# MarioniLab/sarlacc

Hardware: AMD Instinct MI355X
Metric: GCUPS (quality-aware pairwise DP cell updates/s), adaptor_align .Call level (higher is better)
Workload: dtype f64; 1 GPU; adaptorAlign: 1000000 x 2000 bp mockReads-like reads per GPU vs 30 bp adaptor, local quality DP + traceback + 1 section, go=5 ge=1; reads_per_gpu=1000000, read_len=2000, adaptor_len=30, resident_format=2-bit packed bases + 1-bit non-ACGT mask + 1 B quality per base

## Files before the change

### sarlacc_amd/csrc/align.hip

```cpp
#include "align_host.hpp"

#include "../../include/sarlacc_amd.h"

#include <algorithm>
#include <cmath>
#include <cstdlib>
#include <cstring>
#include <limits>

namespace sarlacc {

constexpr int NGMAX = 4;
constexpr int NGMAX2 = 8;
constexpr int NWAVES = 4;
constexpr int RING = 128;
constexpr int RING_MIRROR = 8;
constexpr int RING_SLOT = 256;
constexpr int MAX_REF = 1024;

struct AlignArgs {
    const uint8_t* seq;
    const uint8_t* nmask;
    const uint8_t* qual;
    const int64_t* off;
// ... 14 lines not shown
    const int32_t* sec_e;
    int nsec;
    int32_t* sec_so;
    int32_t* sec_wo;
    void* dirs;
    unsigned long long dirs_per_wave;
    int snap_head, snap_win;
    int* badqual;
    int read_base;
    long long sec_stride;
    uint8_t* aln_ref;
    uint8_t* aln_qry;
    int32_t* aln_len;
    int32_t* edits;
    int wide_maxlen;
    double* wide_bnd;
    int wide_band;
    int* wide_redo;
    const int* wide_list;
    const int* loc_tab;
    const int* loc_rz;
    int loc_GO, loc_GE, loc_D;
    int loc_framed;
    int loc_force;
    double loc_unit, loc_slack, loc_top;
    int* loc_redo;
    int* loc_stats;
    int* loc_out;
    uint8_t* loc_cls;
    int* loc_ccount;
    int* loc_over;
    const int* read_list;
    int bad_done;
};

using mask_t = unsigned long long;
typedef const double __attribute__((address_space(3))) lds_cdouble;
typedef const uint16_t __attribute__((address_space(3))) lds_cu16;
typedef const int __attribute__((address_space(3))) lds_cint;

__device__ __forceinline__ int sel32(int if0, int if1, mask_t m) {
    int r;
    asm("v_cndmask_b32 %0, %1, %2, %3" : "=v"(r) : "v"(if0), "v"(if1), "s"(m));
    return r;
}
__device__ __forceinline__ uint32_t push_bit(uint32_t pk, mask_t m) {
    uint32_t r;
    mask_t carry_out;
    asm("v_addc_co_u32 %0, %1, %2, %2, %3" : "=v"(r), "=s"(carry_out) : "v"(pk), "s"(m));
    return r;
}
__device__ __forceinline__ int hi32(double v) { return static_cast<int>(__double_as_longlong(v) >> 32); }
__device__ __forceinline__ int lo32(double v) { return static_cast<int>(__double_as_longlong(v)); }
__device__ __forceinline__ double mk64(int hi, int lo) {
    return __longlong_as_double((static_cast<long long>(hi) << 32) | static_cast<unsigned int>(lo));
}

template <int ROWF>
__device__ __forceinline__ int lane_shr1(int v, int keep) {
    if (ROWF == 1) return __builtin_amdgcn_update_dpp(keep, v, 0x111 , 0xf, 0xf, false);
    if (ROWF == 2) return __builtin_amdgcn_update_dpp(keep, v, 0x112 , 0xf, 0xf, false);
    return __builtin_amdgcn_update_dpp(v, v, 0x138 , 0xf, 0xf, false);
}
template <int ROWF>
__device__ __forceinline__ double lane_shr1(double v, double keep) {
    return mk64(lane_shr1<ROWF>(hi32(v), hi32(keep)), lane_shr1<ROWF>(lo32(v), lo32(keep)));
}

template <int K>
struct TbSteps { static constexpr int value = (8 / K) > 0 ? 8 / K : 1; };
template <int K>
struct TbStore { using type = uint32_t; };
template <>
struct TbStore<16> { using type = unsigned long long; };

template <bool B>
struct Flag { static constexpr bool value = B; };
template <int V>
struct Int { static constexpr int value = V; };

constexpr int SNAP_P = 64;
static inline int snap_head(int R) { return R + R / 4 + 4; }
static inline int snap_win(int R, int W) { return (SNAP_P + snap_head(R) + W + 7) / 8 * 8; }

constexpr int LOC_NEG = -(1 << 29);
constexpr int LOC_NEG_FRAMED = -(1 << 30);
constexpr int LOC_FRAME_KMIN = 8;
constexpr int LOC_WAVES = 4;
constexpr int LOC_STATS = 6;
constexpr int LOC_NCLS = 32;

struct WinPlan { int ts, want, need; };
__device__ __forceinline__ WinPlan window_plan(const AlignArgs& A, int imax, int lo_x2, int hi_x2) {
    const int lo = (lo_x2 >> 1) + 1, hi = (hi_x2 >> 1) + 1;
    const double f_low = static_cast<double>(imax) * A.loc_unit - A.loc_slack;
    const double over = floor((A.loc_top - f_low) / A.GE) + 1.0;
    const int wc = A.R + (over > 0.0 ? static_cast<int>(fmin(over, 1.0e6)) : 0);
    const int r0 = lo - wc;
    const int ts = r0 < 8 ? 0 : (r0 & ~7);
    return {ts, hi, hi + A.W + 1 - ts};
}

__global__ void __launch_bounds__(256) k_loc_order(const uint8_t* cls, long long n, int* ctl, int* perm) {
    __shared__ int s_cnt[LOC_NCLS], s_base[LOC_NCLS];
    const int t = threadIdx.x;
    if (t < LOC_NCLS) s_cnt[t] = 0;
    __syncthreads();
    const long long read = static_cast<long long>(blockIdx.x) * 256 + t;
    const int c = read < n ? min(static_cast<int>(cls[read]), LOC_NCLS - 1) : 0;
    int rank = 0;
    if (c) rank = atomicAdd(&s_cnt[c], 1);
    __syncthreads();
    if (t < LOC_NCLS) {
        int taller = 0;
        for (int x = t + 1; x < LOC_NCLS; ++x) taller += ctl[x];
        const int mine = t ? s_cnt[t] : 0;
        s_base[t] = taller + (mine ? atomicAdd(&ctl[LOC_NCLS + t], mine) : 0);
        if (blockIdx.x == 0 && t == 0) perm[0] = taller;
    }
    __syncthreads();
    if (c) perm[2 + s_base[c] + rank] = static_cast<int>(read);
}

template <int K, int MODE, bool LOCAL, int ROWF, int KLAST, bool PENSEL>
__global__ void __launch_bounds__(64 * NWAVES, MODE >= 5 ? LOC_WAVES : (MODE == 3 && ROWF != 2) ? 6 : 5) k_align(const AlignArgs A) {
    constexpr bool ROW16 = ROWF != 0;
    constexpr int NG = ROWF == 2 ? NGMAX2 : NGMAX;
    constexpr int SLOT = ROWF == 2 ? RING + RING_MIRROR : RING_SLOT;
    constexpr int UNR = TbSteps<K>::value;
    constexpr int CELLS = UNR * K;
    using Word = typename TbStore<K>::type;
    constexpr bool ADDC = sizeof(Word) == 4;
    extern __shared__ __align__(256) unsigned char smem[];
    static_assert(RING * sizeof(uint16_t) == 256 && RING + RING_MIRROR <= RING_SLOT, "ring addressing assumes 256 B of ring inside a 512 B slot");
    constexpr int RING_BYTES = NWAVES * NG * SLOT * static_cast<int>(sizeof(uint16_t));
    static_assert(RING_BYTES % 8 == 0 && (SLOT * sizeof(uint16_t)) % 8 == 0, "table and 8-byte ring stores stay aligned");
    double* const s_tab = reinterpret_cast<double*>(smem + RING_BYTES);
    const int lds0 = static_cast<int>(reinterpret_cast<size_t>((__attribute__((address_space(3))) unsigned char*)smem));

    const int lane = threadIdx.x & 63;
    const int wave = __builtin_amdgcn_readfirstlane(threadIdx.x >> 6);
    const int W = A.W, R = A.R;
    auto lane_of = [&](int gg, int jj) -> int { return ROWF == 2 ? ((gg >> 1) << 4) + (jj << 1) + (gg & 1) : gg * W + jj; };
    const int g = ROWF == 2 ? (((lane >> 4) << 1) | (lane & 1)) : lane / W;
    const int j = ROWF == 2 ? ((lane & 15) >> 1) : lane - g * W;
    const bool lane_on = g < A.ngroups;
    const bool leader = (j == 0);
    const int c0 = j * K + 1;
    const double NEG_INF = -__builtin_huge_val();
    const double GO = A.GO, GE = A.GE;
    const int GOhi = hi32(GO), GOlo = lo32(GO), GEhi = hi32(GE), GElo = lo32(GE);

    static_assert(MODE < 4 || (ROWF == 2 && LOCAL && !PENSEL), "the locator runs the interleaved local shape only");
    if (A.read_list && A.read_list[0] == 0) return;
    constexpr bool LOCATOR = MODE >= 5, FRAMED = MODE == 6;
    int* const s_tabi = reinterpret_cast<int*>(smem + RING_BYTES);
    if (LOCATOR)
        for (int x = threadIdx.x; x < A.tab_doubles; x += 64 * NWAVES) s_tabi[x] = A.loc_tab[x];
    else
        for (int x = threadIdx.x; x < A.tab_doubles; x += 64 * NWAVES) s_tab[x] = A.tables[x];
    uint16_t* const s_ring = reinterpret_cast<uint16_t*>(smem) + wave * NG * SLOT;
    int32_t* const s_map = reinterpret_cast<int32_t*>(s_tab + A.tab_doubles) + wave * A.ngroups * (R + 1);

    double vgo[K], vge[K], rz[K];
    int colbase[K];
    int colbi[K], vgoi[K], vgei[K], rzi[K];
#pragma unroll
    for (int k = 0; k < K; ++k) {
        const int c = c0 + k;
        const int cc = c <= R ? c : R;
        colbase[k] = lds0 + RING_BYTES + static_cast<int>(A.colbase[cc]);
        const bool last = LOCAL && cc == R && (KLAST < 0 || k == KLAST);
        vgo[k] = last ? 0.0 : GO;
        vge[k] = last ? 0.0 : GE;
        rz[k] = A.rowzero[cc];
        if (LOCATOR) {
            colbi[k] = lds0 + RING_BYTES + static_cast<int>(A.colbase[cc] >> 1);
            vgoi[k] = last ? (FRAMED ? -A.loc_GE : 0) : A.loc_GO;
            vgei[k] = FRAMED ? 0 : last ? 0 : A.loc_GE;
            rzi[k] = A.loc_rz[cc];
        }
    }
    const double rz_left = A.rowzero[c0 - 1 <= R ? c0 - 1 : R];
    const int jlast = (R - 1) / K, klast = KLAST >= 0 ? KLAST : (R - 1) % K;
    const long long gwave = static_cast<long long>(blockIdx.x) * NWAVES + wave;
    const long long nwaves = static_cast<long long>(gridDim.x) * NWAVES;
    Word* const scr = static_cast<Word*>(A.dirs) + static_cast<size_t>(gwave) * A.dirs_per_wave;
    constexpr int NSV = 2 * K + 3;
    double* const snap = reinterpret_cast<double*>(scr + static_cast<size_t>(A.snap_win / UNR) * 64);
    const int ring_g = lds0 + (wave * NG + g) * static_cast<int>(SLOT * sizeof(uint16_t));
    __syncthreads();

    const long long nreads = A.read_list ? static_cast<long long>(A.read_list[0]) : A.n;
    const long long nitems = (nreads + A.ngroups - 1) / A.ngroups;
    int wsteps = 0;
// ... 225 lines not shown
                                    if (is_last && best > V) land_x2 = x2;
                                }
                                if (CODES) {
                                    const unsigned raw = (b_hv ? 1u : 0u) | (b_tm ? 2u : 0u) | (b_hj ? 4u : 0u) | (b_vj ? 8u : 0u);
                                    pk |= static_cast<Word>(raw) << (4 * (CELLS - 1 - (u * K + k)));
                                    if (TR == 1 && is_last) {
                                        const bool cont = b_vj && vnl == 0;
                                        land_up = cont ? land_up : land_prev;
                                        land_prev = vn ? land_up : x2;
                                        vnl = vn ? 1 : 0;
                                    }
                                }
                            }
                        }
                    }
                    if (ROW16 && !LOCAL) {
                        const int i = (x2 >> 1) + 1;
                        const double col0_next = (i < 0) ? 0.0 : (-GO - GE * static_cast<double>(i));
                        s_in = lane_shr1<ROWF>(left, col0_next);
                    } else if (ROW16 && !GUARD) {
                        s_in = lane_shr1<ROWF>(left, s_two_back);
                    } else {
                        s_in = lane_shr1<ROWF>(left, s_in);
                    }
                    lj_in = lane_shr1<ROWF>(lj, lj_in);
                    if (PENSEL) {
                        ph_in = lane_shr1<ROWF>(ph, ph_in);
                        pl_in = lane_shr1<ROWF>(pl, pl_in);
                    }
                    x2 += 2;
                }
                if (TR == 1) __builtin_nontemporal_store(pk, scr + static_cast<size_t>(t0 / UNR) * 64 + lane);
                if (TR == 3 || TR == 5) scr[static_cast<size_t>(t0 / UNR) * 64 + lane] = pk;
            }
            if (!GUARD) vnl = sel32(0, 1, m_vnl);
        };

        const int nsteps = ((Lmax + W + UNR - 1) / UNR) * UNR;
        int t_a = ((W + UNR - 1) / UNR) * UNR;
        int t_b = Lmin == 0x7fffffff ? 0 : ((Lmin + 1) / UNR) * UNR;
        t_a = min(t_a, nsteps);
        t_b = min(max(t_b, t_a), nsteps);
        int loc_max = 0, loc_lo = -2, loc_hi = -2;
        if constexpr (MODE == 4) {
            if (valid && j == jlast) {
                loc_max = A.loc_out[3 * read];
                loc_lo = A.loc_out[3 * read + 1];
                loc_hi = A.loc_out[3 * read + 2];
            }
        } else if constexpr (LOCATOR) {
            int Si[K], Sg[K], UJi[K];
#pragma unroll
            for (int k = 0; k < K; ++k) { Si[k] = rzi[k]; Sg[k] = rzi[k] - vgoi[k]; UJi[k] = LOC_NEG; }
            int si_in = 0, lji_in = LOC_NEG, di_prev = A.loc_rz[c0 - 1 <= R ? c0 - 1 : R];
            const int GOi = A.loc_GO, GEi = A.loc_GE, D = A.loc_D;
            const int D_lo = FRAMED ? D + (UNR - 1) * GEi : D;
            auto run_loc = [&](auto guard_tag, int t_begin, int t_end) {
                constexpr bool GUARD = decltype(guard_tag)::value;
                constexpr int NO_ROW = -0x7fffffff - 1;
                int hi_blk = NO_ROW;
                for (int t0 = t_begin; t0 < t_end; t0 += UNR) {
                    if ((t0 & 63) == 0) {
                        int t0s = t0;
                        asm volatile("" : "+s"(t0s));
#pragma unroll
                        for (int ps = 0; ps < NPASS; ++ps) {
// ... 117 lines not shown
            if (MODE == 4) {
                const int lane_r = lane_of(g, jlast);
                const WinPlan wp = window_plan(A, __shfl(loc_max, lane_r), __shfl(loc_lo, lane_r), __shfl(loc_hi, lane_r));
                ts4 = wp.ts;
                want = wp.want;
                if (valid && (wp.need > A.snap_win || A.loc_force)) {
                    if (leader) push_redo();
                    pending = 0;
                }
            }
            while (__builtin_amdgcn_ballot_w64(pending != 0)) {
                if (--rounds_left < 0) {
                    if (lane == 0) atomicExch(A.badqual + 1, 1);
                    break;
                }
                const int ts = !pending ? 0 : MODE == 4 ? ts4 : (max(want - A.snap_head, 0) / SNAP_P) * SNAP_P;
                int nwin = 0, t_wa = 0, t_wb = 0x7fffffff;
#pragma unroll
                for (int gg = 0; gg < NG; ++gg) {
                    const int src = gg < A.ngroups ? lane_of(gg, 0) : 0;
                    toff[gg] = __builtin_amdgcn_readlane(ts, src);
                    const int pend = __builtin_amdgcn_readlane(pending, src);
                    const int need = __builtin_amdgcn_readlane(want + W + 1 - ts, src);
                    if (gg < A.ngroups && pend) {
                        nwin = max(nwin, need);
                        if (toff[gg] < W) t_wa = W;
                        t_wb = min(t_wb, glen[gg] + 1 - toff[gg]);
                    }
                }
                nwin = min(((nwin + UNR - 1) / UNR) * UNR, A.snap_win);
                if (MODE == 4) wsteps += nwin;
                t_wa = min(((t_wa + UNR - 1) / UNR) * UNR, nwin);
                t_wb = min(max((t_wb / UNR) * UNR, t_wa), nwin);
                __builtin_amdgcn_fence(__ATOMIC_RELEASE, "workgroup");
                __builtin_amdgcn_fence(__ATOMIC_ACQUIRE, "agent");
                if (MODE == 3) {
                    const double* sp = snap + static_cast<size_t>(ts / SNAP_P) * (NSV * 64) + lane;
#pragma unroll
                    for (int k = 0; k < K; ++k) { S[k] = sp[(2 * k) * 64]; UJ[k] = sp[(2 * k + 1) * 64]; }
                    s_in = sp[(2 * K) * 64];
                    lj_in = sp[(2 * K + 1) * 64];
                    diag_prev = sp[(2 * K + 2) * 64];
                } else {
                    const bool fresh = ts > 0;
#pragma unroll
                    for (int k = 0; k < K; ++k) { S[k] = fresh ? NEG_INF : rz[k]; UJ[k] = NEG_INF; }
                    s_in = (fresh && !leader) ? NEG_INF : 0.0;
                    lj_in = NEG_INF;
                    diag_prev = fresh ? (leader ? 0.0 : NEG_INF) : rz_left;
                    land_x2 = -2;
                }
                x2 = 2 * (ts - j - 1);
                x2max = pending ? 2 * L - 2 : -2;
#pragma unroll
                for (int ps = 0; ps < NPASS; ++ps) {
                    const int q = lane >> 4;
                    stoffs[ps] = q == 0 ? toff[4 * ps] : q == 1 ? toff[4 * ps + 1] : q == 2 ? toff[4 * ps + 2] : toff[4 * ps + 3];
                    if (stoffs[ps] >= 64) stage4(sgs[ps], slens[ps], stoffs[ps] - 64, fetch4(slens[ps], sstarts[ps], stoffs[ps] - 64));
                    else if (MODE == 4 && stoffs[ps] > 0) stage4(sgs[ps], slens[ps], 0, fetch4(slens[ps], sstarts[ps], 0));
                    pf[ps] = fetch4(slens[ps], sstarts[ps], stoffs[ps]);
                }
                constexpr int TR_WIN = MODE == 4 ? 5 : 3;
                run(Flag<true>{}, Int<TR_WIN>{}, 0, t_wa);
                run(Flag<false>{}, Int<TR_WIN>{}, t_wa, t_wb);
                run(Flag<true>{}, Int<TR_WIN>{}, t_wb, nwin);
                __builtin_amdgcn_fence(__ATOMIC_RELEASE, "workgroup");
                __builtin_amdgcn_fence(__ATOMIC_ACQUIRE, "agent");
                const int rtop = (MODE == 4 && ts > 0) ? ts : 0;
                if (MODE == 4) {
                    row = (__shfl(land_x2, lane_of(g, jlast)) >> 1) + 1;
                    if (pending && j == jlast) {
                        double sc = S[0];
#pragma unroll
                        for (int k = 1; k < K; ++k) sc = (k == klast) ? S[k] : sc;
                        A.scores[read] = sc;
                    }
                }

                if (pending && leader) {
                    auto code_at = [&](int cc, int rr, unsigned& out) -> bool {
                        const int jj = (cc - 1) / K, kk = (cc - 1) % K;
                        const int tt = rr + jj - ts;
                        if (tt < 0 || rr < rtop) return false;
                        const Word w = wtile[static_cast<size_t>(tt / UNR) * 64 + lane_of(g, jj)];
                        out = static_cast<unsigned>(w >> (4 * (CELLS - 1 - ((tt % UNR) * K + kk)))) & 15u;
                        return true;
                    };
                    bool stalled = false;
                    while (c > 0 && !stalled) {
                        if (phase == 0) {
                            while (c > 0 && row > 0) {
                                const int jj = (c - 1) / K, kk = (c - 1) % K;
                                const int tt = row + jj - ts;
                                if (tt < 0 || row < rtop) break;
                                const Word w = wtile[static_cast<unsigned>(tt / UNR) * 64u + static_cast<unsigned>(lane_of(g, jj))];
                                if (!((w >> (4 * (CELLS - 1 - ((tt % UNR) * K + kk)))) & 2u)) break;
                                map[c] = row * 2 + 1;
                                --row; --c;
                            }
                            if (c <= 0) break;
                            if (row <= 0) { map[c] = (row + 1) * 2; --c; continue; }
                            unsigned nb;
                            if (!code_at(c, row, nb)) { want = row; stalled = true; break; }
                            if (nb & 2u) { map[c] = row * 2 + 1; --row; --c; continue; }
                            cur = nb;
                            chain_n = 0;
                            phase = (nb & 1u) ? 1 : 2;
                            chain_at = (nb & 1u) ? c : row;
                        }
                        if (phase == 1) {
                            while ((cur & 4u) && chain_at > 1) {
                                unsigned prev;
                                if (!code_at(chain_at - 1, row, prev)) { want = row; stalled = true; break; }
                                if ((prev & 3u) == 1u) break;
                                ++chain_n; --chain_at; cur = prev;
                            }
                            if (stalled) break;
                            for (int x = 0; x <= chain_n; ++x) { map[c] = (row + 1) * 2; --c; }
                            phase = 0;
                        } else {
                            while ((cur & 8u) && chain_at > 1) {
                                unsigned prev;
                                if (!code_at(c, chain_at - 1, prev)) { want = chain_at - 1; stalled = true; break; }
                                if ((prev & 3u) == 0u) break;
                                ++chain_n; --chain_at; cur = prev;
                            }
                            if (stalled) break;
                            row -= 1 + chain_n;
                            phase = 0;
                        }
                    }
                    if (MODE == 4 && stalled) {
                        atomicAdd(A.loc_stats + 1, 1);
                        push_redo();
                        pending = 0;
                    }
                    if (!stalled) {
                        pending = 0;
                        auto interval = [&](int a, int b, bool gaps, unsigned& s, unsigned& e) {
                            if (!gaps) {
                                s = map[a + 1] >> 1;
                                e = (map[b] >> 1) + (map[b] & 1);
                            } else {
                                s = (a == 0) ? 1u : static_cast<unsigned>((map[a] >> 1) + (map[a] & 1));
                                e = (b + 1 == R + 1) ? static_cast<unsigned>(L + 1) : static_cast<unsigned>(map[b + 1] >> 1);
                            }
                            s -= 1;
                            e -= 1;
                        };
                        unsigned s, e;
                        interval(0, R, false, s, e);
                        const bool nonempty = s < e;
                        A.starts[read] = nonempty ? static_cast<int32_t>(s + 1) : 0;
                        A.ends[read] = nonempty ? static_cast<int32_t>(e) : 0;
                        for (int x = 0; x < A.nsec; ++x) {
                            interval(A.sec_s[x], A.sec_e[x], true, s, e);
                            A.sec_so[static_cast<long long>(x) * A.sec_stride + read] = static_cast<int32_t>(s + 1);
                            A.sec_wo[static_cast<long long>(x) * A.sec_stride + read] = static_cast<int32_t>(e - s);
                        }
                    }
                }
                pending = __shfl(pending, lane_of(g, 0));
                want = __shfl(want, lane_of(g, 0));
            }
        }

        if (MODE == 1 || MODE == 2) {
            __builtin_amdgcn_fence(__ATOMIC_RELEASE, "workgroup");
            __builtin_amdgcn_fence(__ATOMIC_ACQUIRE, "agent");
            const int land = (__shfl(land_prev, lane_of(g, jlast)) >> 1) + 1;
            if (valid && leader) {
// ... 56 lines not shown
                        A.sec_so[static_cast<long long>(x) * A.sec_stride + read] = static_cast<int32_t>(s + 1);
                        A.sec_wo[static_cast<long long>(x) * A.sec_stride + read] = static_cast<int32_t>(e - s);
                    }
                } else {
                    const long long base = start + read * static_cast<long long>(R);
                    uint8_t* oref = A.aln_ref + base;
                    uint8_t* oqry = A.aln_qry + base;
                    const uint8_t* sq = A.seq + start;
                    int m = 0, ed = 0;
                    for (; row > land; --row) { oref[m] = '-'; oqry[m] = sq[row - 1]; ++m; ++ed; }
                    while (c > 0) {
                        int d = loadD(c, row);
                        while (row > 0 && d < 0) {
                            for (int x = 0; x < -d; ++x) { oref[m] = '-'; oqry[m] = sq[row - 1]; ++m; ++ed; --row; }
                            d = loadD(c, row);
                        }
                        if (d == 0) {
                            const uint8_t rc = A.refchars[c - 1], qc = sq[row - 1];
                            oref[m] = rc; oqry[m] = qc; ++m;
                            ed += rc != qc;
                            --row; --c;
                        } else {
                            for (int x = 0; x < d; ++x) { oref[m] = A.refchars[c - 1]; oqry[m] = '-'; ++m; ++ed; --c; }
                        }
                    }
                    while (row > 0) { oref[m] = '-'; oqry[m] = sq[row - 1]; ++m; ++ed; --row; }
                    A.aln_len[read] = m;
                    A.edits[read] = ed;
                }
            }
        }
    }
    if (MODE == 4 && lane == 0 && wsteps) atomicAdd(reinterpret_cast<unsigned long long*>(A.loc_stats + 4), static_cast<unsigned long long>(wsteps));
}

__global__ void k_align_emptyref(const int64_t* off, long long n, int local, double GO, double GE,
                                 double* scores, int32_t* starts, int32_t* ends, int nsec,
                                 int32_t* sec_so, int32_t* sec_wo, int32_t* aln_len, int32_t* edits,
                                 const uint8_t* seq, uint8_t* aln_ref, uint8_t* aln_qry) {
    const long long r = blockIdx.x * static_cast<long long>(blockDim.x) + threadIdx.x;
    if (r >= n) return;
    const int L = static_cast<int>(off[r + 1] - off[r]);
    scores[r] = (local || L < 1) ? 0.0 : (-GO - GE * static_cast<double>(L - 1));
    if (starts) { starts[r] = 0; ends[r] = 0; }
    for (int x = 0; x < nsec; ++x) { sec_so[x * n + r] = 1; sec_wo[x * n + r] = 0; }
    if (aln_len) {
        for (int m = 0; m < L; ++m) { aln_ref[off[r] + m] = '-'; aln_qry[off[r] + m] = seq[off[r] + L - 1 - m]; }
        aln_len[r] = L;
        edits[r] = L;
    }
}

constexpr int WIDE_CH = 512;
constexpr int WIDE_RING = 2048;
constexpr int WIDE_MAXT = 1024;

template <int K>
struct WideWord { using type = uint32_t; };

struct WideBand {
    int band, L, R;
    __device__ __forceinline__ int lo(int w) const { return static_cast<int>(512ll * w * L / R) - band - 2; }
    __device__ __forceinline__ int hi(int w) const { return static_cast<int>((512ll * (w + 1) * L + R - 1) / R) + band + 64; }
    __device__ __forceinline__ bool stored(int c, int row) const {
        if (band <= 0) return true;
        const int t = (c - 1) >> 3, w = t >> 6, sg = row + (t & 63) - 1;
// ... 706 lines not shown
    if (mode == 0 && local) hipLaunchKernelGGL((k_align<K, 0, true, ROW16, KLAST, PENSEL>), dim3(grid), dim3(64 * NWAVES), lds, s, a);
    else if (mode == 0) hipLaunchKernelGGL((k_align<K, 0, false, ROW16, KLAST, PENSEL>), dim3(grid), dim3(64 * NWAVES), lds, s, a);
    else if (mode == 1 && local) hipLaunchKernelGGL((k_align<K, 1, true, ROW16, KLAST, PENSEL>), dim3(grid), dim3(64 * NWAVES), lds, s, a);
    else if (mode == 3 && local && !PENSEL) hipLaunchKernelGGL((k_align<K, 3, true, ROW16, KLAST, false>), dim3(grid), dim3(64 * NWAVES), lds, s, a);
    else if (mode == 2 && !local) hipLaunchKernelGGL((k_align<K, 2, false, ROW16, KLAST, PENSEL>), dim3(grid), dim3(64 * NWAVES), lds, s, a);
    else return fail("sarlacc_amd: unsupported alignment mode");
    SL_HIP(hipGetLastError());
    return 0;
}

template <int K, int ROW16, int KLAST>
static int launch_pen(bool pensel, int mode, bool local, const AlignArgs& a, int grid, size_t lds, hipStream_t s) {
    return pensel ? launch_mode<K, ROW16, KLAST, true>(mode, local, a, grid, lds, s)
                  : launch_mode<K, ROW16, KLAST, false>(mode, local, a, grid, lds, s);
}

struct LocLaunch {
    int* order = nullptr;
    void* redo_dirs = nullptr;
    unsigned long long redo_per_wave = 0;
    int redo_grid = 0;
    hipStream_t side = nullptr;
    hipEvent_t fork = nullptr, join = nullptr;
};

template <int K, int KLAST>
static int launch_il(int mode, const AlignArgs& a, int grid, size_t lds, hipStream_t s, const LocLaunch* ll) {
    if (mode == 4) {
        const size_t lds5 = sizeof(uint16_t) * NWAVES * NGMAX2 * (RING + RING_MIRROR) + sizeof(int) * a.tab_doubles + 16;
        if (a.loc_framed) hipLaunchKernelGGL((k_align<K, 6, true, 2, KLAST, false>), dim3(grid), dim3(64 * NWAVES), lds5, s, a);
        else hipLaunchKernelGGL((k_align<K, 5, true, 2, KLAST, false>), dim3(grid), dim3(64 * NWAVES), lds5, s, a);
        AlignArgs r = a;
        r.bad_done = 1;
        if (!ll) {
            hipLaunchKernelGGL((k_align<K, 4, true, 2, KLAST, false>), dim3(grid), dim3(64 * NWAVES), lds, s, a);
            r.read_list = a.loc_redo;
            hipLaunchKernelGGL((k_align<K, 3, true, 2, KLAST, false>), dim3(grid), dim3(64 * NWAVES), lds, s, r);
        } else {
            r.dirs = ll->redo_dirs;
            r.dirs_per_wave = ll->redo_per_wave;
            SL_HIP(hipEventRecord(ll->fork, s));
            SL_HIP(hipStreamWaitEvent(ll->side, ll->fork, 0));
            r.read_list = a.loc_over;
            hipLaunchKernelGGL((k_align<K, 3, true, 2, KLAST, false>), dim3(ll->redo_grid), dim3(64 * NWAVES), lds, ll->side, r);
            SL_HIP(hipEventRecord(ll->join, ll->side));
            hipLaunchKernelGGL(k_loc_order, dim3(static_cast<unsigned>((a.n + 255) / 256)), dim3(256), 0, s, a.loc_cls, a.n, a.loc_ccount, ll->order);
            AlignArgs w = a;
            w.read_list = ll->order;
            w.bad_done = 1;
            hipLaunchKernelGGL((k_align<K, 4, true, 2, KLAST, false>), dim3(grid), dim3(64 * NWAVES), lds, s, w);
            SL_HIP(hipStreamWaitEvent(s, ll->join, 0));
            r.read_list = a.loc_redo;
            hipLaunchKernelGGL((k_align<K, 3, true, 2, KLAST, false>), dim3(ll->redo_grid), dim3(64 * NWAVES), lds, s, r);
        }
    } else if (mode == 3) hipLaunchKernelGGL((k_align<K, 3, true, 2, KLAST, false>), dim3(grid), dim3(64 * NWAVES), lds, s, a);
    else hipLaunchKernelGGL((k_align<K, 0, true, 2, KLAST, false>), dim3(grid), dim3(64 * NWAVES), lds, s, a);
    SL_HIP(hipGetLastError());
    return 0;
}

static int launch_k(int K, int rowf, int R, bool pensel, int mode, bool local, const AlignArgs& a, int grid, size_t lds,
                    hipStream_t s, const LocLaunch* ll = nullptr) {
    const int klast = (R - 1) % K;
    if (rowf == 2) {
        if (!local || pensel || !(mode == 3 || mode == 4 || mode == 0)) return fail("sarlacc_amd: interleaved alignments serve local modes 0 and 3 only");
        const int key = K * 4 + klast;
        switch (key) {
            case 2 * 4 + 0: return launch_il<2, 0>(mode, a, grid, lds, s, ll);
            case 2 * 4 + 1: return launch_il<2, 1>(mode, a, grid, lds, s, ll);
            case 4 * 4 + 0: return launch_il<4, 0>(mode, a, grid, lds, s, ll);
            case 4 * 4 + 1: return launch_il<4, 1>(mode, a, grid, lds, s, ll);
            case 4 * 4 + 2: return launch_il<4, 2>(mode, a, grid, lds, s, ll);
            case 4 * 4 + 3: return launch_il<4, 3>(mode, a, grid, lds, s, ll);
        }
        return fail("sarlacc_amd: unsupported columns-per-lane %d for interleaved alignments", K);
    }
    const bool row16 = rowf == 1;
    if (K == 1) return row16 ? launch_pen<1, 1, 0>(pensel, mode, local, a, grid, lds, s) : launch_pen<1, 0, 0>(pensel, mode, local, a, grid, lds, s);
    if (K == 2) {
        if (row16) return klast == 0 ? launch_pen<2, 1, 0>(pensel, mode, local, a, grid, lds, s) : launch_pen<2, 1, 1>(pensel, mode, local, a, grid, lds, s);
        return klast == 0 ? launch_pen<2, 0, 0>(pensel, mode, local, a, grid, lds, s) : launch_pen<2, 0, 1>(pensel, mode, local, a, grid, lds, s);
    }
    switch (K) {
// ... 220 lines not shown
            SL_TRY(upload("align.lstats", zero, LOC_STATS, &d_stats, stream));
            if (!co.finish) SL_HIP(hipStreamSynchronize(stream));
        } else {
            SL_TRY(scratch("align.ltab", lp.tab.size(), &d_ltab));
            SL_TRY(scratch("align.lrz", lp.rz.size(), &d_lrz));
            SL_TRY(scratch("align.lstats", LOC_STATS, &d_stats));
        }
        SL_TRY(scratch("align.lredo", static_cast<size_t>(n) + 2, &d_redo));
        SL_TRY(scratch("align.lout", static_cast<size_t>(n) * 3, &a.loc_out));
        SL_HIP(hipMemsetAsync(d_redo, 0, 2 * sizeof(int), stream));
        a.loc_tab = d_ltab; a.loc_rz = d_lrz; a.loc_redo = d_redo; a.loc_stats = d_stats;
        a.loc_GO = lp.GO; a.loc_GE = lp.GE; a.loc_D = lp.D; a.loc_force = option(OPT_ALIGN_LOCATE) == 1 ? 1 : 0;
        a.loc_framed = lp.framed ? 1 : 0;
        a.loc_unit = lp.unit; a.loc_slack = lp.slack; a.loc_top = lp.top;
        if (classes) {
            SL_TRY(scratch("align.lcls", static_cast<size_t>(n), &a.loc_cls));
            SL_TRY(scratch("align.lccount", static_cast<size_t>(2 * LOC_NCLS), &d_ccount));
            SL_TRY(scratch("align.lover", static_cast<size_t>(n) + 2, &a.loc_over));
            SL_TRY(scratch("align.lorder", static_cast<size_t>(n) + 2, &ll.order));
            SL_HIP(hipMemsetAsync(d_ccount, 0, 2 * LOC_NCLS * sizeof(int), stream));
            SL_HIP(hipMemsetAsync(a.loc_over, 0, 2 * sizeof(int), stream));
            a.loc_ccount = d_ccount;
            const size_t wg_bytes = std::max<size_t>(1, redo_per_wave * word_bytes * NWAVES);
            ll.redo_grid = static_cast<int>(std::max<size_t>(1, std::min<size_t>((c.num_cu + 3) / 4, (static_cast<size_t>(6) << 30) / wg_bytes)));
            ll.redo_per_wave = redo_per_wave;
            SL_TRY(c.buffer("align.rdirs", static_cast<size_t>(ll.redo_grid) * wg_bytes, &ll.redo_dirs));
            SL_TRY(c.side_stream(&ll.side, &ll.fork, &ll.join));
        }
    }

    const size_t lds = sizeof(uint16_t) * NWAVES * (sh.rowf == 2 ? NGMAX2 * (RING + RING_MIRROR) : NGMAX * RING_SLOT) + sizeof(double) * rows.size() +
                       sizeof(int32_t) * NWAVES * sh.ngroups * (R + 1) + 16;
    if (!wide && lds > 64 * 1024) return fail("sarlacc_amd: alignment tables do not fit in LDS");
    if (co.stage) SL_TRY(c.stage_begin(co.stage, stream));
    else SL_HIP(hipEventRecord(c.ev_start, stream));
    if (wide) SL_TRY(launch_wide(a, R, kernel_mode == 3 ? 1 : kernel_mode, max_len, n, stream));
    else SL_TRY(launch_k(sh.K, sh.rowf, R, pensel, kernel_mode, local, a, static_cast<int>(grid), lds, stream, classes ? &ll : nullptr));
    if (co.stage) {
        SL_TRY(c.stage_end(co.stage, stream));
    } else {
        SL_HIP(hipEventRecord(c.ev_stop, stream));
        c.timed = true;
    }

    if (!co.finish) return 0;
    int flags[2] = {0, 0}, lstats[LOC_STATS] = {}, ccount[LOC_NCLS] = {};
    SL_HIP(hipMemcpyAsync(flags, d_bad, sizeof flags, hipMemcpyDeviceToHost, stream));
    if (d_stats) SL_HIP(hipMemcpyAsync(lstats, d_stats, sizeof lstats, hipMemcpyDeviceToHost, stream));
    if (d_ccount) SL_HIP(hipMemcpyAsync(ccount, d_ccount, sizeof ccount, hipMemcpyDeviceToHost, stream));
    SL_HIP(hipStreamSynchronize(stream));
    *bad_qual_read = flags[0];
    if (kernel_mode == 3 || kernel_mode == 4) {
        c.counts["align_redo"] = d_stats ? lstats[0] : -1.0;
        c.counts["align_stalls"] = d_stats ? lstats[1] : -1.0;
        c.counts["align_oversize"] = d_stats ? lstats[2] : -1.0;
        unsigned long long wsteps = 0;
        std::memcpy(&wsteps, lstats + 4, sizeof wsteps);
        c.counts["align_window_steps"] = d_stats ? static_cast<double>(wsteps) : -1.0;
        static const std::vector<std::string> class_keys = [] {
            std::vector<std::string> v;
            for (int x = 0; x < LOC_NCLS; ++x) v.push_back("align_window_class_" + std::to_string(x));
            return v;
        }();
        for (int x = 1; x < LOC_NCLS; ++x) c.counts[class_keys[x]] = d_ccount ? ccount[x] : -1.0;
        c.counts["align_locate_k"] = d_stats ? (lp.framed ? lp.k : -lp.k) : 0.0;
    }
    if (flags[1]) return fail("sarlacc_amd: internal error: an alignment traceback exceeded its bound");
    return 0;
}

int first_error(int64_t n, const int64_t* seq_off, const int64_t* qual_off, const char* ref, int R,
                int bad_qual_read) {
    int64_t len_bad = -1;
    if (qual_off)
        for (int64_t i = 0; i < n; ++i)
            if (seq_off[i + 1] - seq_off[i] != qual_off[i + 1] - qual_off[i]) { len_bad = i; break; }
    int first_bad_col = -1;
    uint32_t tmp;
    for (int col = 0; col < R; ++col)
        if (column_info(ref[col], &tmp)) { first_bad_col = col; break; }
    int64_t first_nonempty = -1;
    if (first_bad_col >= 0)
        for (int64_t i = 0; i < n; ++i)
            if (seq_off[i + 1] - seq_off[i] > 0) { first_nonempty = i; break; }

    const int64_t INF = std::numeric_limits<int64_t>::max();
    const int64_t e_len = len_bad >= 0 ? len_bad : INF;
    const int64_t e_qual = (R > 0 && bad_qual_read != std::numeric_limits<int>::max()) ? bad_qual_read : INF;
    const int64_t e_ref = first_nonempty >= 0 ? first_nonempty : INF;
    const int64_t first = std::min(e_len, std::min(e_qual, e_ref));
    if (first == INF) return 0;
// ... 287 lines not shown
```

### sarlacc_amd/csrc/common.cpp

```cpp
#include "common.hpp"

#include <algorithm>
#include <vector>

#include <cstdlib>

#include "../../include/sarlacc_amd.h"

namespace sarlacc {

std::string& last_error() {
    static thread_local std::string msg;
    return msg;
}

int fail(const char* fmt, ...) {
    char buf[512];
    va_list ap;
    va_start(ap, fmt);
    vsnprintf(buf, sizeof buf, fmt, ap);
    va_end(ap);
    last_error() = buf;
    return 1;
}

static const char* const kOptNames[OPT_N] = {"msa_spec", "msa2_general_rows", "msa2_chain_hbm", "msa2_waves_per_cu", "msa2_single_wave", "msa2_batches", "align_pensel", "align_chunks",
                                             "align_k", "align_waves_per_cu", "consensus_chars", "consensus_generic", "msa_int32", "msa_affine", "umi_full_rounds", "umi_tile_search", "msa_bitvector", "msa_bitvector_core", "msa_bitvector_tile_gb", "align_interleave", "umi_split_min", "msa2_tight_profiles", "umi_scan_single", "align_wide_barrier", "msa2_budget_gb", "msa2_max_columns", "align_wide_band", "msa2_simple_extend", "msa2_wide_extend", "align_locate", "align_panel", "profile_chunk_reads", "align_window_classes"};
static int* option_values() {
    static int values[OPT_N];
    static const bool parsed = [] {
        for (int k = 0; k < OPT_N; ++k) {
            std::string env = "SARLACC_";
            for (const char* p = kOptNames[k]; *p; ++p) env += static_cast<char>(*p >= 'a' && *p <= 'z' ? *p - 32 : *p);
            const char* e = std::getenv(env.c_str());
            values[k] = e ? std::atoi(e) : 0;
        }
        return true;
    }();
    (void)parsed;
    return values;
}
int option(Opt o) { return option_values()[o]; }
int set_option(const char* name, int value) {
    for (int k = 0; k < OPT_N; ++k)
        if (name && std::strcmp(name, kOptNames[k]) == 0) { option_values()[k] = value; return 0; }
    return fail("sarlacc_amd: unknown option '%s'", name ? name : "(null)");
}

Context& ctx() {
    static thread_local Context c;
    return c;
}

int ensure_device() {
    Context& c = ctx();
    if (c.ready) {
        SL_HIP(hipSetDevice(c.device));
        return 0;
    }
    int count = 0;
// ... 193 lines not shown
```

### sarlacc_amd/csrc/common.hpp

```cpp
#pragma once

#include <hip/hip_runtime.h>

#include <cstdarg>
#include <cstdint>
#include <cstdio>
#include <cstring>
#include <functional>
#include <map>
#include <string>
#include <vector>

namespace sarlacc {

std::string& last_error();
int fail(const char* fmt, ...);

#define SL_HIP(expr)                                                              \
    do {                                                                          \
        hipError_t e__ = (expr);                                                  \
        if (e__ != hipSuccess)                                                    \
            return ::sarlacc::fail("HIP error %s at %s:%d (%s)", hipGetErrorName(e__), \
                                   __FILE__, __LINE__, #expr);                    \
    } while (0)
// ... 8 lines not shown
    OPT_MSA_SPEC,
    OPT_MSA2_GENERAL_ROWS,
    OPT_MSA2_CHAIN_HBM,
    OPT_MSA2_WAVES_PER_CU,
    OPT_MSA2_SINGLE_WAVE,
    OPT_MSA2_BATCHES,
    OPT_ALIGN_PENSEL,
    OPT_ALIGN_CHUNKS,
    OPT_ALIGN_K,
    OPT_ALIGN_WAVES_PER_CU,
    OPT_CONSENSUS_CHARS,
    OPT_CONSENSUS_GENERIC,
    OPT_MSA_INT32,
    OPT_MSA_AFFINE,
    OPT_UMI_FULL_ROUNDS,
    OPT_UMI_TILE_SEARCH,
    OPT_MSA_BITVECTOR,
    OPT_MSA_BITVECTOR_CORE,
    OPT_MSA_BITVECTOR_TILE_GB,
    OPT_ALIGN_INTERLEAVE,
    OPT_UMI_SPLIT_MIN,
    OPT_MSA2_TIGHT_PROFILES,
    OPT_UMI_SCAN_SINGLE,
    OPT_ALIGN_WIDE_BARRIER,
    OPT_MSA2_BUDGET_GB,
    OPT_MSA2_MAX_COLUMNS,
    OPT_ALIGN_WIDE_BAND,
    OPT_MSA2_SIMPLE_EXTEND,
    OPT_MSA2_WIDE_EXTEND,
    OPT_ALIGN_LOCATE,
    OPT_ALIGN_PANEL,
    OPT_PROFILE_CHUNK_READS,
    OPT_ALIGN_WINDOW_CLASSES,
    OPT_N
};
int option(Opt o);
int set_option(const char* name, int value);

struct Workspace {
    void* ptr = nullptr;
    size_t cap = 0;
};

struct Context {
    int device = 0;
    bool ready = false;
    int num_cu = 0;
    hipEvent_t ev_start = nullptr, ev_stop = nullptr;
    enum { TIMED_PANEL = 2 };
    int timed = 0;
    std::map<std::string, Workspace> ws;
    struct StageTimer { std::vector<std::pair<hipEvent_t, hipEvent_t>> segs; size_t used = 0; bool open = false; };
    std::map<std::string, StageTimer> stages;
    std::map<std::string, double> counts;
    hipStream_t side = nullptr;
    hipEvent_t ev_fork = nullptr, ev_join = nullptr;
    int side_stream(hipStream_t* s, hipEvent_t* fork, hipEvent_t* join);
    void side_release();
    void stage_reset(const char* name);
    int stage_begin(const char* name, hipStream_t s);
    int stage_end(const char* name, hipStream_t s);

    int buffer(const char* name, size_t bytes, void** out);
    int64_t release_matching(const std::function<bool(const std::string&)>& match);
    void release();
};
// ... 49 lines not shown
```

Baseline: 3466 GCUPS.

## Keep recent window traceback codes in an LDS ring and walk diagonals wave-wide

For the MODE 4 window kernel, each wave also writes its traceback code words into a per-wave LDS ring sized to the expected walk depth. The traceback then reads from LDS and falls back to global memory, with the agent-scope fence taken lazily, only when the walk leaves the ring. The diagonal phase of the walk now uses all eight lanes of a group with a ballot to advance up to eight cells per step instead of a leader-only serial loop. This trades extra LDS (fewer waves per CU via launch bounds 3) and extra LDS stores in the DP loop for avoiding global reads and fences on the traceback, and adds counters for ring misses.

```diff
diff --git a/sarlacc_amd/csrc/align.hip b/sarlacc_amd/csrc/align.hip
--- a/sarlacc_amd/csrc/align.hip
+++ b/sarlacc_amd/csrc/align.hip
@@ -70,6 +70,7 @@
     int* loc_over;
     const int* read_list;
     int bad_done;
+    int win_nb;
 };
 
 using mask_t = unsigned long long;
@@ -125,7 +126,9 @@
 constexpr int LOC_NEG_FRAMED = -(1 << 30);
 constexpr int LOC_FRAME_KMIN = 8;
 constexpr int LOC_WAVES = 4;
-constexpr int LOC_STATS = 6;
+constexpr int LOC_STATS = 8;
+constexpr int WIN_LDS_WAVES = 3;
+static inline int win_ring_blocks(int R, int W, int unr) { return (snap_head(R) + W + unr - 1) / unr + 1; }
 constexpr int LOC_NCLS = 32;
 
 struct WinPlan { int ts, want, need; };
@@ -160,8 +163,8 @@
     if (c) perm[2 + s_base[c] + rank] = static_cast<int>(read);
 }
 
-template <int K, int MODE, bool LOCAL, int ROWF, int KLAST, bool PENSEL>
-__global__ void __launch_bounds__(64 * NWAVES, MODE >= 5 ? LOC_WAVES : (MODE == 3 && ROWF != 2) ? 6 : 5) k_align(const AlignArgs A) {
+template <int K, int MODE, bool LOCAL, int ROWF, int KLAST, bool PENSEL, bool WLDS = false>
+__global__ void __launch_bounds__(64 * NWAVES, WLDS ? WIN_LDS_WAVES : MODE >= 5 ? LOC_WAVES : (MODE == 3 && ROWF != 2) ? 6 : 5) k_align(const AlignArgs A) {
     constexpr bool ROW16 = ROWF != 0;
     constexpr int NG = ROWF == 2 ? NGMAX2 : NGMAX;
     constexpr int SLOT = ROWF == 2 ? RING + RING_MIRROR : RING_SLOT;
@@ -190,6 +193,7 @@
     const int GOhi = hi32(GO), GOlo = lo32(GO), GEhi = hi32(GE), GElo = lo32(GE);
 
     static_assert(MODE < 4 || (ROWF == 2 && LOCAL && !PENSEL), "the locator runs the interleaved local shape only");
+    static_assert(!WLDS || MODE == 4, "the LDS code ring belongs to the MODE 4 window");
     if (A.read_list && A.read_list[0] == 0) return;
     constexpr bool LOCATOR = MODE >= 5, FRAMED = MODE == 6;
     int* const s_tabi = reinterpret_cast<int*>(smem + RING_BYTES);
@@ -199,6 +203,11 @@
         for (int x = threadIdx.x; x < A.tab_doubles; x += 64 * NWAVES) s_tab[x] = A.tables[x];
     uint16_t* const s_ring = reinterpret_cast<uint16_t*>(smem) + wave * NG * SLOT;
     int32_t* const s_map = reinterpret_cast<int32_t*>(s_tab + A.tab_doubles) + wave * A.ngroups * (R + 1);
+    const int code_ring_bytes = WLDS ? A.win_nb * 64 * static_cast<int>(sizeof(Word)) : 0;
+    unsigned char* const s_code = reinterpret_cast<unsigned char*>(reinterpret_cast<int32_t*>(s_tab + A.tab_doubles) + NWAVES * A.ngroups * (R + 1)) +
+                                  wave * code_ring_bytes;
+    int code_ofs = 0;
+    int walk_glob = 0, walks_out = 0;
 
     double vgo[K], vge[K], rz[K];
     int colbase[K];
@@ -490,6 +499,11 @@
                 }
                 if (TR == 1) __builtin_nontemporal_store(pk, scr + static_cast<size_t>(t0 / UNR) * 64 + lane);
                 if (TR == 3 || TR == 5) scr[static_cast<size_t>(t0 / UNR) * 64 + lane] = pk;
+                if (TR == 5 && WLDS) {
+                    *reinterpret_cast<Word*>(s_code + code_ofs + lane * static_cast<int>(sizeof(Word))) = pk;
+                    code_ofs += 64 * static_cast<int>(sizeof(Word));
+                    if (code_ofs == code_ring_bytes) code_ofs = 0;
+                }
             }
             if (!GUARD) vnl = sel32(0, 1, m_vnl);
         };
@@ -673,8 +687,11 @@
                 if (MODE == 4) wsteps += nwin;
                 t_wa = min(((t_wa + UNR - 1) / UNR) * UNR, nwin);
                 t_wb = min(max((t_wb / UNR) * UNR, t_wa), nwin);
-                __builtin_amdgcn_fence(__ATOMIC_RELEASE, "workgroup");
-                __builtin_amdgcn_fence(__ATOMIC_ACQUIRE, "agent");
+                if (!WLDS) {
+                    __builtin_amdgcn_fence(__ATOMIC_RELEASE, "workgroup");
+                    __builtin_amdgcn_fence(__ATOMIC_ACQUIRE, "agent");
+                }
+                code_ofs = 0;
                 if (MODE == 3) {
                     const double* sp = snap + static_cast<size_t>(ts / SNAP_P) * (NSV * 64) + lane;
 #pragma unroll
@@ -705,8 +722,15 @@
                 run(Flag<true>{}, Int<TR_WIN>{}, 0, t_wa);
                 run(Flag<false>{}, Int<TR_WIN>{}, t_wa, t_wb);
                 run(Flag<true>{}, Int<TR_WIN>{}, t_wb, nwin);
-                __builtin_amdgcn_fence(__ATOMIC_RELEASE, "workgroup");
-                __builtin_amdgcn_fence(__ATOMIC_ACQUIRE, "agent");
+                if (WLDS) {
+                    __builtin_amdgcn_fence(__ATOMIC_ACQ_REL, "wavefront");
+                } else {
+                    __builtin_amdgcn_fence(__ATOMIC_RELEASE, "workgroup");
+                    __builtin_amdgcn_fence(__ATOMIC_ACQUIRE, "agent");
+                }
+                const int last_blk = nwin / UNR - 1;
+                const int last_ofs = (code_ofs ? code_ofs : code_ring_bytes) - 64 * static_cast<int>(sizeof(Word));
+                bool tile_fenced = false;
                 const int rtop = (MODE == 4 && ts > 0) ? ts : 0;
                 if (MODE == 4) {
                     row = (__shfl(land_x2, lane_of(g, jlast)) >> 1) + 1;
@@ -718,26 +742,66 @@
                     }
                 }
 
-                if (pending && leader) {
+                constexpr bool GWALK = WLDS;
+                if (pending && (GWALK || leader)) {
+                    auto tile_word = [&](int tt, int ln, bool counted) -> Word {
+                        const unsigned b = static_cast<unsigned>(tt) / UNR;
+                        if (WLDS) {
+                            const unsigned back = static_cast<unsigned>(last_blk) - b;
+                            if (back < static_cast<unsigned>(A.win_nb)) {
+                                int o = last_ofs - static_cast<int>(back) * 64 * static_cast<int>(sizeof(Word));
+                                o += o < 0 ? code_ring_bytes : 0;
+                                return *reinterpret_cast<const Word*>(s_code + o + ln * static_cast<int>(sizeof(Word)));
+                            }
+                            if (!tile_fenced) {
+                                __builtin_amdgcn_fence(__ATOMIC_RELEASE, "workgroup");
+                                __builtin_amdgcn_fence(__ATOMIC_ACQUIRE, "agent");
+                                tile_fenced = true;
+                            }
+                            walk_glob += counted ? 1 : 0;
+                        }
+                        return wtile[b * 64u + static_cast<unsigned>(ln)];
+                    };
                     auto code_at = [&](int cc, int rr, unsigned& out) -> bool {
                         const int jj = (cc - 1) / K, kk = (cc - 1) % K;
                         const int tt = rr + jj - ts;
                         if (tt < 0 || rr < rtop) return false;
-                        const Word w = wtile[static_cast<size_t>(tt / UNR) * 64 + lane_of(g, jj)];
+                        const Word w = tile_word(tt, lane_of(g, jj), leader);
                         out = static_cast<unsigned>(w >> (4 * (CELLS - 1 - ((tt % UNR) * K + kk)))) & 15u;
                         return true;
                     };
                     bool stalled = false;
                     while (c > 0 && !stalled) {
                         if (phase == 0) {
-                            while (c > 0 && row > 0) {
+                            while (!GWALK && c > 0 && row > 0) {
                                 const int jj = (c - 1) / K, kk = (c - 1) % K;
                                 const int tt = row + jj - ts;
                                 if (tt < 0 || row < rtop) break;
-                                const Word w = wtile[static_cast<unsigned>(tt / UNR) * 64u + static_cast<unsigned>(lane_of(g, jj))];
+                                const Word w = tile_word(tt, lane_of(g, jj), true);
                                 if (!((w >> (4 * (CELLS - 1 - ((tt % UNR) * K + kk)))) & 2u)) break;
                                 map[c] = row * 2 + 1;
                                 --row; --c;
+                            }
+                            while (GWALK && c > 0 && row > 0) {
+                                const int rr = row - j, cc = c - j;
+                                bool on = false;
+                                if (cc > 0 && rr > 0) {
+                                    const int jj = (cc - 1) / K, kk = (cc - 1) % K;
+                                    const int tt = rr + jj - ts;
+                                    if (tt >= 0 && rr >= rtop) {
+                                        const Word w = tile_word(tt, lane_of(g, jj), true);
+                                        on = ((w >> (4 * (CELLS - 1 - ((tt % UNR) * K + kk)))) & 2u) != 0;
+                                    }
+                                }
+                                const mask_t off_m = __builtin_amdgcn_ballot_w64(!on);
+                                unsigned x = static_cast<unsigned>(off_m >> lane_of(g, 0)) & 0x5555u;
+                                x = (x | (x >> 1)) & 0x3333u;
+                                x = (x | (x >> 2)) & 0x0f0fu;
+                                x = (x | (x >> 4)) & 0xffu;
+                                const int len = __builtin_ctz(x | 0x100u);
+                                if (j < len) map[cc] = rr * 2 + 1;
+                                row -= len; c -= len;
+                                if (len < 8) break;
                             }
                             if (c <= 0) break;
                             if (row <= 0) { map[c] = (row + 1) * 2; --c; continue; }
@@ -771,13 +835,19 @@
                             phase = 0;
                         }
                     }
+                    if (GWALK) {
+                        const mask_t out_m = __builtin_amdgcn_ballot_w64(tile_fenced);
+                        if (leader && ((out_m >> lane_of(g, 0)) & 0x5555u)) ++walks_out;
+                    }
                     if (MODE == 4 && stalled) {
-                        atomicAdd(A.loc_stats + 1, 1);
-                        push_redo();
+                        if (leader) {
+                            atomicAdd(A.loc_stats + 1, 1);
+                            push_redo();
+                        }
                         pending = 0;
                     }
-                    if (!stalled) {
-                        pending = 0;
+                    if (!stalled) pending = 0;
+                    if (!stalled && leader) {
                         auto interval = [&](int a, int b, bool gaps, unsigned& s, unsigned& e) {
                             if (!gaps) {
                                 s = map[a + 1] >> 1;
@@ -900,6 +970,8 @@
         }
     }
     if (MODE == 4 && lane == 0 && wsteps) atomicAdd(reinterpret_cast<unsigned long long*>(A.loc_stats + 4), static_cast<unsigned long long>(wsteps));
+    if (WLDS && walks_out) atomicAdd(A.loc_stats + 3, walks_out);
+    if (WLDS && walk_glob) atomicAdd(reinterpret_cast<unsigned long long*>(A.loc_stats + 6), static_cast<unsigned long long>(walk_glob));
 }
 
 __global__ void k_align_emptyref(const int64_t* off, long long n, int local, double GO, double GE,
@@ -1672,8 +1744,23 @@
         else hipLaunchKernelGGL((k_align<K, 5, true, 2, KLAST, false>), dim3(grid), dim3(64 * NWAVES), lds5, s, a);
         AlignArgs r = a;
         r.bad_done = 1;
+        const size_t lds4 = lds + static_cast<size_t>(NWAVES) * a.win_nb * 64 * sizeof(uint32_t);
+        auto windows = [&](const AlignArgs& w) -> int {
+            if (!a.win_nb) {
+                hipLaunchKernelGGL((k_align<K, 4, true, 2, KLAST, false>), dim3(grid), dim3(64 * NWAVES), lds, s, w);
+                return 0;
+            }
+            static thread_local size_t lds_set = 0;
+            if (lds4 > 48 * 1024 && lds4 > lds_set) {
+                SL_HIP(hipFuncSetAttribute(reinterpret_cast<const void*>(&k_align<K, 4, true, 2, KLAST, false, true>),
+                                           hipFuncAttributeMaxDynamicSharedMemorySize, static_cast<int>(lds4)));
+                lds_set = lds4;
+            }
+            hipLaunchKernelGGL((k_align<K, 4, true, 2, KLAST, false, true>), dim3(grid), dim3(64 * NWAVES), lds4, s, w);
+            return 0;
+        };
         if (!ll) {
-            hipLaunchKernelGGL((k_align<K, 4, true, 2, KLAST, false>), dim3(grid), dim3(64 * NWAVES), lds, s, a);
+            SL_TRY(windows(a));
             r.read_list = a.loc_redo;
             hipLaunchKernelGGL((k_align<K, 3, true, 2, KLAST, false>), dim3(grid), dim3(64 * NWAVES), lds, s, r);
         } else {
@@ -1688,7 +1775,7 @@
             AlignArgs w = a;
             w.read_list = ll->order;
             w.bad_done = 1;
-            hipLaunchKernelGGL((k_align<K, 4, true, 2, KLAST, false>), dim3(grid), dim3(64 * NWAVES), lds, s, w);
+            SL_TRY(windows(w));
             SL_HIP(hipStreamWaitEvent(s, ll->join, 0));
             r.read_list = a.loc_redo;
             hipLaunchKernelGGL((k_align<K, 3, true, 2, KLAST, false>), dim3(ll->redo_grid), dim3(64 * NWAVES), lds, s, r);
@@ -1975,6 +2062,16 @@
     const size_t lds = sizeof(uint16_t) * NWAVES * (sh.rowf == 2 ? NGMAX2 * (RING + RING_MIRROR) : NGMAX * RING_SLOT) + sizeof(double) * rows.size() +
                        sizeof(int32_t) * NWAVES * sh.ngroups * (R + 1) + 16;
     if (!wide && lds > 64 * 1024) return fail("sarlacc_amd: alignment tables do not fit in LDS");
+    int win_nb = 0;
+    if (kernel_mode == 4 && option(OPT_ALIGN_WINDOW_LDS) >= 0) {
+        const int tile_blocks = snap_win(R, sh.W) / tb_steps;
+        win_nb = option(OPT_ALIGN_WINDOW_LDS) >= 2 ? option(OPT_ALIGN_WINDOW_LDS) : win_ring_blocks(R, sh.W, tb_steps);
+        win_nb = std::min(win_nb, tile_blocks);
+        const size_t block_bytes = static_cast<size_t>(NWAVES) * 64 * sizeof(uint32_t);
+        win_nb = static_cast<int>(std::min<size_t>(win_nb, (64 * 1024 - lds) / block_bytes));
+        if (win_nb < 2) win_nb = 0;
+    }
+    a.win_nb = win_nb;
     if (co.stage) SL_TRY(c.stage_begin(co.stage, stream));
     else SL_HIP(hipEventRecord(c.ev_start, stream));
     if (wide) SL_TRY(launch_wide(a, R, kernel_mode == 3 ? 1 : kernel_mode, max_len, n, stream));
@@ -2000,6 +2097,10 @@
         unsigned long long wsteps = 0;
         std::memcpy(&wsteps, lstats + 4, sizeof wsteps);
         c.counts["align_window_steps"] = d_stats ? static_cast<double>(wsteps) : -1.0;
+        unsigned long long wglob = 0;
+        std::memcpy(&wglob, lstats + 6, sizeof wglob);
+        c.counts["align_walk_global"] = d_stats && win_nb ? static_cast<double>(wglob) : -1.0;
+        c.counts["align_walk_left_ring"] = d_stats && win_nb ? lstats[3] : -1.0;
         static const std::vector<std::string> class_keys = [] {
             std::vector<std::string> v;
             for (int x = 0; x < LOC_NCLS; ++x) v.push_back("align_window_class_" + std::to_string(x));
diff --git a/sarlacc_amd/csrc/common.cpp b/sarlacc_amd/csrc/common.cpp
--- a/sarlacc_amd/csrc/common.cpp
+++ b/sarlacc_amd/csrc/common.cpp
@@ -25,7 +25,7 @@
 }
 
 static const char* const kOptNames[OPT_N] = {"msa_spec", "msa2_general_rows", "msa2_chain_hbm", "msa2_waves_per_cu", "msa2_single_wave", "msa2_batches", "align_pensel", "align_chunks",
-                                             "align_k", "align_waves_per_cu", "consensus_chars", "consensus_generic", "msa_int32", "msa_affine", "umi_full_rounds", "umi_tile_search", "msa_bitvector", "msa_bitvector_core", "msa_bitvector_tile_gb", "align_interleave", "umi_split_min", "msa2_tight_profiles", "umi_scan_single", "align_wide_barrier", "msa2_budget_gb", "msa2_max_columns", "align_wide_band", "msa2_simple_extend", "msa2_wide_extend", "align_locate", "align_panel", "profile_chunk_reads", "align_window_classes"};
+                                             "align_k", "align_waves_per_cu", "consensus_chars", "consensus_generic", "msa_int32", "msa_affine", "umi_full_rounds", "umi_tile_search", "msa_bitvector", "msa_bitvector_core", "msa_bitvector_tile_gb", "align_interleave", "umi_split_min", "msa2_tight_profiles", "umi_scan_single", "align_wide_barrier", "msa2_budget_gb", "msa2_max_columns", "align_wide_band", "msa2_simple_extend", "msa2_wide_extend", "align_locate", "align_panel", "profile_chunk_reads", "align_window_classes", "align_window_lds"};
 static int* option_values() {
     static int values[OPT_N];
     static const bool parsed = [] {
diff --git a/sarlacc_amd/csrc/common.hpp b/sarlacc_amd/csrc/common.hpp
--- a/sarlacc_amd/csrc/common.hpp
+++ b/sarlacc_amd/csrc/common.hpp
@@ -64,6 +64,7 @@
     OPT_ALIGN_PANEL,
     OPT_PROFILE_CHUNK_READS,
     OPT_ALIGN_WINDOW_CLASSES,
+    OPT_ALIGN_WINDOW_LDS,
     OPT_N
 };
 int option(Opt o);
```

Measured after the change: 3685 GCUPS, median of 6. 6.3% higher.
